# atenpas/gpd

Measured on AMD Instinct MI355X. Metric: 15-ch grasp candidates scored/sec (imagegen+LeNet) at 1/2/4/8 MI355X, higher is better.
Workload: dtype f64 geometry / u8 images / LeNet f32-equivalent by exact operand splitting: conv1 int8 digit planes of 32-bit fixed-point weights (i32 accumulate, exact), conv2 + ip1 three bf16 pieces per operand (six exact products per term, f32 accumulate), ip2 f32

## Files before the change

### gpd_amd/csrc/lenet_fast.hip

```cpp
#include "gpd_internal.h"
#include "buffers.h"

#include <cstring>

namespace gpd {

typedef int i32x4 __attribute__((ext_vector_type(4)));
typedef float f32x4 __attribute__((ext_vector_type(4)));
typedef __bf16 bf16x8 __attribute__((ext_vector_type(8)));
typedef unsigned int u32x4 __attribute__((ext_vector_type(4)));

constexpr int F1_THREADS = 512, F1_WAVES = 8;
constexpr int F1_PITCH = 72;
constexpr int F1_ROWB = F1_PITCH * 16;
constexpr int F1_HWC = kImg * F1_ROWB;
constexpr int F1_TILES = 28 * 7;
constexpr int F1_KS = 7, F1_MT = 5;

__host__ __device__ constexpr int f1_tap(int ks, int g) {
  return ks < 5 ? ((g == 0 ? 0 : g == 1 ? 2 : g == 2 ? 1 : 3) * 5 + ks) : ks == 5 ? 20 + g : (g == 0 ? 24 : -1);
}
constexpr int F1P_KS = 5;
constexpr int F1P_ROWB = 736;
constexpr int F1P_COPY = kImg * F1P_ROWB;
constexpr int F1N_KS = 3;
constexpr int F1N_PITCH = 68;
constexpr int F1N_COPY = kImg * F1N_PITCH * 4;
__host__ __device__ constexpr int f1n_slot(int ks, int g) {
  const int sl = 4 * ks + g;
  return sl < 5 ? 2 * sl : sl < 10 ? 2 * (sl - 5) + 1 : -1;
}

__device__ inline double max_f64(double a, double b) {
  double r;
  asm("v_max_f64 %0, %1, %2" : "=v"(r) : "v"(a), "v"(b));
  return r;
}
__device__ inline double dpp_quad_max(double v) {
  int lo = __double2loint(v), hi = __double2hiint(v);
  double o = __hiloint2double(__builtin_amdgcn_mov_dpp(hi, 0xB1, 0xf, 0xf, true), __builtin_amdgcn_mov_dpp(lo, 0xB1, 0xf, 0xf, true));
  v = max_f64(v, o);
  lo = __double2loint(v);
  hi = __double2hiint(v);
  o = __hiloint2double(__builtin_amdgcn_mov_dpp(hi, 0x4E, 0xf, 0xf, true), __builtin_amdgcn_mov_dpp(lo, 0x4E, 0xf, 0xf, true));
  return max_f64(v, o);
}

template <int C, bool RELU>
__device__ __forceinline__ void conv1_i8_body(const uint8_t *__restrict__ images, const uint4 *__restrict__ atab,
                                              const double *__restrict__ corr, const int *__restrict__ shift,
                                              const float *__restrict__ bias, float *__restrict__ pool1, int n,
                                              int *__restrict__ queue) {
  constexpr int RAW = C * kPix, NV = RAW / 16;
  static_assert(RAW % 16 == 0 && C <= 16, "image bytes");
  constexpr bool NARROW = C <= 4;
  constexpr bool PACK12 = C == 12;
  constexpr int KS = NARROW ? F1N_KS : PACK12 ? F1P_KS : F1_KS;
  __shared__ __attribute__((aligned(16))) uint8_t s_hwc[NARROW ? 4 * F1N_COPY : PACK12 ? 2 * F1P_COPY : F1_HWC];
  __shared__ __attribute__((aligned(16))) uint8_t s_raw[RAW];
  __shared__ int s_nxt;
  const int tid = threadIdx.x, lane = tid & 63;
  const int wave = __builtin_amdgcn_readfirstlane(tid >> 6);
  const int j = lane & 15, q = lane >> 4;
  int img = blockIdx.x;
  if (img >= n) return;
  if (wave < F1_WAVES / 2) __builtin_amdgcn_s_setprio(2);
  i32x4 A[KS][F1_MT];
#pragma unroll
  for (int ks = 0; ks < KS; ks++)
#pragma unroll
    for (int mt = 0; mt < F1_MT; mt++) {
      const uint4 v = atab[(ks * F1_MT + mt) * 64 + lane];
      A[ks][mt] = i32x4{(int)v.x, (int)v.y, (int)v.z, (int)v.w};
    }
  {
    const uint4 *src = reinterpret_cast<const uint4 *>(images + (size_t)img * RAW);
    uint4 *dst = reinterpret_cast<uint4 *>(s_raw);
    for (int i = tid; i < NV; i += F1_THREADS) dst[i] = src[i];
  }
  __syncthreads();
  auto transpose = [&]() {
    if constexpr (NARROW) {
      for (int task = tid; task < kImg * (kImg / 4); task += F1_THREADS) {
        const int y = task / (kImg / 4), x0 = 4 * (task - y * (kImg / 4));
        uint32_t r[4];
#pragma unroll
        for (int c = 0; c < 4; c++) r[c] = c < C ? *reinterpret_cast<const uint32_t *>(s_raw + c * kPix + y * kImg + x0) : 0x80808080u;
        const uint32_t t0 = __builtin_amdgcn_perm(r[1], r[0], 0x05010400u), t1 = __builtin_amdgcn_perm(r[1], r[0], 0x07030602u);
        const uint32_t t2 = __builtin_amdgcn_perm(r[3], r[2], 0x05010400u), t3 = __builtin_amdgcn_perm(r[3], r[2], 0x07030602u);
        const uint32_t o0 = __builtin_amdgcn_perm(t2, t0, 0x05040100u) ^ 0x80808080u, o1 = __builtin_amdgcn_perm(t2, t0, 0x07060302u) ^ 0x80808080u;
        const uint32_t o2 = __builtin_amdgcn_perm(t3, t1, 0x05040100u) ^ 0x80808080u, o3 = __builtin_amdgcn_perm(t3, t1, 0x07060302u) ^ 0x80808080u;
        uint8_t *d = s_hwc + (y * F1N_PITCH + x0) * 4;
        *reinterpret_cast<uint4 *>(d) = make_uint4(o0, o1, o2, o3);
#pragma unroll
        for (int sh = 1; sh < 4; sh++) {
          uint32_t *e = reinterpret_cast<uint32_t *>(d + sh * F1N_COPY + sh * 4);
          e[0] = o0;
          e[1] = o1;
          e[2] = o2;
          e[3] = o3;
        }
      }
      return;
    }
    if constexpr (PACK12) {
      for (int task = tid; task < kImg * (kImg / 4); task += F1_THREADS) {
        const int y = task / (kImg / 4), x0 = 4 * (task - y * (kImg / 4));
        uint32_t o[4][3];
#pragma unroll
        for (int cg = 0; cg < 3; cg++) {
          uint32_t r[4];
#pragma unroll
          for (int c = 0; c < 4; c++) r[c] = *reinterpret_cast<const uint32_t *>(s_raw + (4 * cg + c) * kPix + y * kImg + x0);
          const uint32_t t0 = __builtin_amdgcn_perm(r[1], r[0], 0x05010400u), t1 = __builtin_amdgcn_perm(r[1], r[0], 0x07030602u);
          const uint32_t t2 = __builtin_amdgcn_perm(r[3], r[2], 0x05010400u), t3 = __builtin_amdgcn_perm(r[3], r[2], 0x07030602u);
          o[0][cg] = __builtin_amdgcn_perm(t2, t0, 0x05040100u) ^ 0x80808080u;
          o[1][cg] = __builtin_amdgcn_perm(t2, t0, 0x07060302u) ^ 0x80808080u;
          o[2][cg] = __builtin_amdgcn_perm(t3, t1, 0x05040100u) ^ 0x80808080u;
          o[3][cg] = __builtin_amdgcn_perm(t3, t1, 0x07060302u) ^ 0x80808080u;
        }
        uint8_t *d = s_hwc + y * F1P_ROWB + 12 * x0;
        uint4 *d4 = reinterpret_cast<uint4 *>(d);
        d4[0] = make_uint4(o[0][0], o[0][1], o[0][2], o[1][0]);
        d4[1] = make_uint4(o[1][1], o[1][2], o[2][0], o[2][1]);
        d4[2] = make_uint4(o[2][2], o[3][0], o[3][1], o[3][2]);
        uint32_t *e = reinterpret_cast<uint32_t *>(d + F1P_COPY + 4);
#pragma unroll
        for (int px = 0; px < 4; px++)
#pragma unroll
          for (int cg = 0; cg < 3; cg++) e[3 * px + cg] = o[px][cg];
      }
      return;
    }
    for (int task = tid; task < kImg * (kImg / 4); task += F1_THREADS) {
      const int y = task / (kImg / 4), x0 = 4 * (task - y * (kImg / 4));
      uint32_t r[16];
#pragma unroll
      for (int c = 0; c < 16; c++) r[c] = c < C ? *reinterpret_cast<const uint32_t *>(s_raw + c * kPix + y * kImg + x0) : 0u;
      uint32_t o[4][4];
#pragma unroll
      for (int cg = 0; cg < 4; cg++) {
        const uint32_t t0 = __builtin_amdgcn_perm(r[4 * cg + 1], r[4 * cg], 0x05010400u);
        const uint32_t t1 = __builtin_amdgcn_perm(r[4 * cg + 1], r[4 * cg], 0x07030602u);
        const uint32_t t2 = __builtin_amdgcn_perm(r[4 * cg + 3], r[4 * cg + 2], 0x05010400u);
        const uint32_t t3 = __builtin_amdgcn_perm(r[4 * cg + 3], r[4 * cg + 2], 0x07030602u);
        o[0][cg] = __builtin_amdgcn_perm(t2, t0, 0x05040100u) ^ 0x80808080u;
        o[1][cg] = __builtin_amdgcn_perm(t2, t0, 0x07060302u) ^ 0x80808080u;
        o[2][cg] = __builtin_amdgcn_perm(t3, t1, 0x05040100u) ^ 0x80808080u;
        o[3][cg] = __builtin_amdgcn_perm(t3, t1, 0x07060302u) ^ 0x80808080u;
      }
#pragma unroll
      for (int e = 0; e < 4; e++)
        *reinterpret_cast<uint4 *>(s_hwc + (y * F1_PITCH + x0 + e) * 16) = make_uint4(o[e][0], o[e][1], o[e][2], o[e][3]);
    }
  };
  transpose();
  const int m_row = (j >> 1) & 1, m_x = 2 * (j >> 2) + (j & 1);
  const int kyg = q == 0 ? 0 : q == 1 ? 2 : q == 2 ? 1 : 3;
  const int n_shift = (4 - (m_x & 3)) & 3;
  const int lane_off = NARROW   ? n_shift * F1N_COPY + (m_row * F1N_PITCH + m_x + n_shift) * 4
                       : PACK12 ? (m_x & 1) * (F1P_COPY + 4) + m_row * F1P_ROWB + 12 * m_x + 16 * q
                                : (m_row * F1_PITCH + m_x) * 16;
  int n_slot[F1N_KS];
#pragma unroll
  for (int ks = 0; ks < F1N_KS; ks++) {
    const int sl = q == 0 ? f1n_slot(ks, 0) : q == 1 ? f1n_slot(ks, 1) : q == 2 ? f1n_slot(ks, 2) : f1n_slot(ks, 3);
    n_slot[ks] = sl < 0 ? 0 : ((sl >> 1) * F1N_PITCH + 4 * (sl & 1)) * 4;
  }
  const int p = j & 3, w = j >> 2;
  const double k_corr_own = corr[4 * p + q], k_corr_4 = corr[16 + q];
  const int k_shift_own = shift[4 * p + q], k_shift_4 = shift[16 + q];
  const float k_bias_own = bias[4 * p + q], k_bias_4 = bias[16 + q];
  for (;;) {
    if (tid == 0) s_nxt = (int)gridDim.x + atomicAdd(queue, 1);
    __syncthreads();
    const int nxt = s_nxt;
    const uint4 *nsrc = reinterpret_cast<const uint4 *>(images + (size_t)(nxt < n ? nxt : img) * RAW);
    auto tile_addr = [&](int t, const uint8_t *&pa, const uint8_t *&pb, const uint8_t *&pc) {
      const int tc = t < F1_TILES ? t : F1_TILES - 1;
      const int trow = tc / 7, tcol = tc - 7 * trow;
      if constexpr (NARROW) {
        pa = pb = pc = s_hwc + ((2 * trow) * F1N_PITCH + 8 * tcol) * 4 + lane_off;
      } else if constexpr (PACK12) {
        pa = pb = pc = s_hwc + (2 * trow) * F1P_ROWB + 12 * (8 * tcol) + lane_off;
      } else {
        const uint8_t *base = s_hwc + ((2 * trow) * F1_PITCH + 8 * tcol) * 16 + lane_off;
        pa = base + kyg * F1_ROWB;
        pb = base + 4 * F1_ROWB + q * 16;
        pc = base + 4 * F1_ROWB + 4 * 16;
      }
    };
    auto frag_b = [&](int ks, const uint8_t *pa, const uint8_t *pb, const uint8_t *pc) {
      if constexpr (NARROW) return *reinterpret_cast<const i32x4 *>(pa + n_slot[ks < F1N_KS ? ks : 0]);
      else if constexpr (PACK12) {
        typedef const volatile __attribute__((address_space(3))) unsigned long long *lds_u64;
        const unsigned long long lo = *(lds_u64)(pa + ks * F1P_ROWB), hi = *(lds_u64)(pa + ks * F1P_ROWB + 8);
        return i32x4{(int)(uint32_t)lo, (int)(uint32_t)(lo >> 32), (int)(uint32_t)hi, (int)(uint32_t)(hi >> 32)};
      }
      else return *reinterpret_cast<const i32x4 *>(ks < 5 ? pa + ks * 16 : ks == 5 ? pb : pc);
    };
    i32x4 B[KS];
    {
      const uint8_t *pa, *pb, *pc;
      tile_addr(wave, pa, pb, pc);
#pragma unroll
      for (int ks = 0; ks < KS; ks++) B[ks] = frag_b(ks, pa, pb, pc);
    }
    int it = 0;
    for (int t = wave; t < F1_TILES; t += F1_WAVES, it++) {
      const int piece = it * F1_THREADS + tid;
      const bool has_piece = nxt < n && piece < NV;
      uint4 stage = make_uint4(0, 0, 0, 0);
      if (has_piece) stage = nsrc[piece];
      i32x4 acc[F1_MT];
#pragma unroll
      for (int mt = 0; mt < F1_MT; mt++) acc[mt] = i32x4{0, 0, 0, 0};
      __builtin_amdgcn_sched_barrier(0);
#pragma unroll
      for (int ks = 0; ks < KS; ks++)
#pragma unroll
        for (int mt = 0; mt < F1_MT; mt++) acc[mt] = __builtin_amdgcn_mfma_i32_16x16x64_i8(A[ks][mt], B[ks], acc[mt], 0, 0, 0);
      __builtin_amdgcn_sched_barrier(0);
      {
        const uint8_t *pa, *pb, *pc;
        tile_addr(t + F1_WAVES, pa, pb, pc);
#pragma unroll
        for (int ks = 0; ks < KS; ks++) B[ks] = frag_b(ks, pa, pb, pc);
      }
      __builtin_amdgcn_sched_barrier(0);
      double sm[F1_MT];
#pragma unroll
      for (int mt = 0; mt < F1_MT; mt++) {
        const int hi = (int)((unsigned)acc[mt][3] << 8) + acc[mt][2];
        const int lo = (int)((unsigned)acc[mt][1] << 8) + acc[mt][0];
        sm[mt] = dpp_quad_max(__builtin_fma((double)hi, 65536.0, (double)lo));
      }
      const double s_own = p == 0 ? sm[0] : p == 1 ? sm[1] : p == 2 ? sm[2] : sm[3];
      float v_own = ldexpf((float)(s_own + k_corr_own), -k_shift_own) + k_bias_own;
      float v_4 = ldexpf((float)(sm[4] + k_corr_4), -k_shift_4) + k_bias_4;
      if constexpr (RELU) {
        v_own = fmaxf(v_own, 0.f);
        v_4 = fmaxf(v_4, 0.f);
      }
      const int trow = t / 7, tcol = t - 7 * trow;
      float *dst = pool1 + ((size_t)img * 784 + trow * 28 + 4 * tcol + w) * 20;
      dst[4 * p + q] = v_own;
      if (p == 0) dst[16 + q] = v_4;
      if (has_piece) reinterpret_cast<uint4 *>(s_raw)[piece] = stage;
    }
    __syncthreads();
    if (nxt >= n) break;
    transpose();
    img = nxt;
  }
}

template <int C>
__global__ __launch_bounds__(F1_THREADS) void conv1_i8_kernel(const uint8_t *__restrict__ images,
                                                              const uint4 *__restrict__ atab, const double *__restrict__ corr,
                                                              const int *__restrict__ shift, const float *__restrict__ bias,
                                                              float *__restrict__ pool1, int n, int *__restrict__ queue) {
  conv1_i8_body<C, false>(images, atab, corr, shift, bias, pool1, n, queue);
}
template <int C>
__global__ __launch_bounds__(F1_THREADS) void conv1_i8_relu_kernel(const uint8_t *__restrict__ images,
                                                                   const uint4 *__restrict__ atab,
                                                                   const double *__restrict__ corr,
                                                                   const int *__restrict__ shift,
                                                                   const float *__restrict__ bias, float *__restrict__ pool1,
                                                                   int n, int *__restrict__ queue) {
  conv1_i8_body<C, true>(images, atab, corr, shift, bias, pool1, n, queue);
}

__device__ inline bf16x8 as_bf16x8(const uint4 &v) {
  bf16x8 r;
  __builtin_memcpy(&r, &v, 16);
  return r;
}

struct Bf3 {
  unsigned short h, m, l;
};
__host__ __device__ inline unsigned short bf16_bits(float x) {
#if defined(__HIP_DEVICE_COMPILE__)
  const __bf16 b = (__bf16)x;
  unsigned short u;
  __builtin_memcpy(&u, &b, 2);
  return u;
#else
  uint32_t u;
  memcpy(&u, &x, 4);
  if ((u & 0x7f800000u) == 0x7f800000u) return (unsigned short)((u >> 16) | ((u & 0xffffu) ? 0x40u : 0u));
  u += 0x7fffu + ((u >> 16) & 1u);
  return (unsigned short)(u >> 16);
#endif
}
__host__ __device__ inline float bf16_value(unsigned short b) {
  const uint32_t u = (uint32_t)b << 16;
  float f;
#if defined(__HIP_DEVICE_COMPILE__)
  __builtin_memcpy(&f, &u, 4);
#else
  memcpy(&f, &u, 4);
#endif
  return f;
}
__host__ __device__ inline Bf3 bf16_split3(float a) {
  Bf3 r;
  r.h = bf16_bits(a);
  const float r1 = a - bf16_value(r.h);
  r.m = bf16_bits(r1);
  const float r2 = r1 - bf16_value(r.m);
  r.l = bf16_bits(r2);
  return r;
}

constexpr int F2_THREADS = 512;
constexpr int F2_PP = 28 * 40;
constexpr int F2_RS = 3 * F2_PP;
constexpr int F2_IMG = 28 * F2_RS;
constexpr int F2_RAW = 784 * 20 * 4;
constexpr int F2_LUNITS = 24;
constexpr int F2_XLD = kLenetXld;

constexpr int F3_KSTEPS = F2_XLD / 32;
__host__ __device__ inline size_t f3_blocked(int r, int k, int pc) {
  const int rr = r & 15;
  return ((((size_t)(r >> 4) * F3_KSTEPS + (k >> 5)) * 3 + pc) << 10) + rr * 64 + ((((k >> 3) & 3) ^ ((4 - (rr >> 2)) & 3)) << 4) + (k & 7) * 2;
}

__host__ __device__ constexpr int f2_slot_tap(int e, int g) {
  return e < 25 ? (e / 5) * 5 + g : e < 30 ? g * 5 + 4 : e == 30 ? 24 : (g == 0 ? 24 : -1);
}
__host__ __device__ constexpr int f2_slot_cg(int e, int g) { return e < 25 ? e % 5 : e < 30 ? e - 25 : e == 30 ? g : 4; }

template <bool RELU>
__device__ __forceinline__ void conv2_bf16_body(const float *__restrict__ pool1, const uint4 *__restrict__ btab,
                                                const float *__restrict__ bias, unsigned short *__restrict__ xs, int n,
                                                int *__restrict__ queue) {
  __shared__ __attribute__((aligned(16))) uint8_t s_img[F2_IMG];
  __shared__ __attribute__((aligned(16))) uint8_t s_raw[F2_RAW];
  __shared__ int s_nxt;
  const int tid = threadIdx.x, lane = tid & 63;
  const int wave = __builtin_amdgcn_readfirstlane(tid >> 6);
  const int j = lane & 15, q = lane >> 4;
  const int img0 = blockIdx.x;
  if (img0 >= n) return;
  {
    const uint4 *src = reinterpret_cast<const uint4 *>(pool1 + (size_t)img0 * (784 * 20));
    uint4 *dst = reinterpret_cast<uint4 *>(s_raw);
    for (int i = tid; i < F2_RAW / 16; i += F2_THREADS) dst[i] = src[i];
  }
  __syncthreads();
  auto split = [&]() {
    for (int task = tid; task < 784 * 5; task += F2_THREADS) {
      const int px = task / 5, cg = task - 5 * px;
      const int row = px / 28, col = px - 28 * row;
      const float4 a = *reinterpret_cast<const float4 *>(s_raw + px * 80 + cg * 16);
      const Bf3 s0 = bf16_split3(a.x), s1 = bf16_split3(a.y), s2 = bf16_split3(a.z), s3 = bf16_split3(a.w);
      uint8_t *d = s_img + row * F2_RS + col * 40 + cg * 8;
      *reinterpret_cast<uint2 *>(d) = make_uint2(s0.h | ((uint32_t)s1.h << 16), s2.h | ((uint32_t)s3.h << 16));
      *reinterpret_cast<uint2 *>(d + F2_PP) = make_uint2(s0.m | ((uint32_t)s1.m << 16), s2.m | ((uint32_t)s3.m << 16));
      *reinterpret_cast<uint2 *>(d + 2 * F2_PP) = make_uint2(s0.l | ((uint32_t)s1.l << 16), s2.l | ((uint32_t)s3.l << 16));
    }
  };
  split();
  auto store_x = [&](int img, int pixel, int f, float v) {
    const Bf3 sp = bf16_split3(v);
    uint8_t *o = reinterpret_cast<uint8_t *>(xs) + f3_blocked(img, pixel * 50 + f, 0);
    *reinterpret_cast<unsigned short *>(o) = sp.h;
    *reinterpret_cast<unsigned short *>(o + 1024) = sp.m;
    *reinterpret_cast<unsigned short *>(o + 2048) = sp.l;
  };
  auto image_loop = [&](int passes, auto carries, auto &&work) {
    int img = img0;
    for (;;) {
      if (tid == 0) s_nxt = (int)gridDim.x + atomicAdd(queue, 1);
      __syncthreads();
      const int nxt = s_nxt;
      const uint4 *nsrc = reinterpret_cast<const uint4 *>(pool1 + (size_t)(nxt < n ? nxt : img) * (784 * 20));
#pragma unroll 1
      for (int tt = 0; tt < passes; tt++) {
        const int piece = tt * (7 * 64) + tid;
        const bool has_piece = decltype(carries)::value && nxt < n && piece < F2_RAW / 16;
        uint4 stage = make_uint4(0, 0, 0, 0);
        if (has_piece) stage = nsrc[piece];
        work(img, tt);
        if (has_piece) reinterpret_cast<uint4 *>(s_raw)[piece] = stage;
      }
      __syncthreads();
      if (nxt >= n) break;
      split();
      img = nxt;
    }
  };
  if (wave == 7) {
    __builtin_amdgcn_s_setprio(3);
    bf16x8 LW[3][4];
#pragma unroll
    for (int pc = 0; pc < 3; pc++)
#pragma unroll
      for (int ks = 0; ks < 4; ks++) LW[pc][ks] = as_bf16x8(btab[((3 * 3 + pc) * 16 + ks) * 64 + lane]);
    int l_lo[4], l_hi[4];
#pragma unroll
    for (int ks = 0; ks < 4; ks++) {
      const int idx = min(4 * ks + q, 14), ky = idx / 3, c8 = idx - 3 * ky;
      l_lo[ks] = ky * F2_RS + j * 40 + c8 * 16;
      l_hi[ks] = c8 == 2 ? l_lo[ks] : l_lo[ks] + 8;
    }
    const int f_own = 48 + (q & 1);
    const float k_bias = bias[f_own];
    auto unit_base = [&](int u) { return s_img + (2 * (u >> 1)) * F2_RS + (12 * (u & 1)) * 40; };
    auto lfrag = [&](const uint8_t *ubase, int step, int pc) -> bf16x8 {
      typedef const volatile __attribute__((address_space(3))) unsigned long long *lds_u64;
      const uint8_t *a = ubase + (step >> 2) * F2_RS + pc * F2_PP;
      const unsigned long long lo = *(lds_u64)(a + l_lo[step & 3]), hi = *(lds_u64)(a + l_hi[step & 3]);
      return as_bf16x8(make_uint4((uint32_t)lo, (uint32_t)(lo >> 32), (uint32_t)hi, (uint32_t)(hi >> 32)));
    };
    bf16x8 b_buf[4][3];
    auto shl = [](float v, auto n) {
      return __builtin_bit_cast(float, __builtin_amdgcn_update_dpp(0, __builtin_bit_cast(int, v), 0x100 + decltype(n)::value, 0xf, 0xf, true));
    };
    asm volatile("" ::"v"(k_bias));
    image_loop(F2_LUNITS, std::false_type(), [&](int img, int tt) {
      const uint8_t *ubase = unit_base(tt), *unext = unit_base(tt < F2_LUNITS - 1 ? tt + 1 : tt);
      if (tt == 0) {
#pragma unroll
        for (int st = 0; st < 3; st++)
#pragma unroll
          for (int pc = 0; pc < 3; pc++) b_buf[st][pc] = lfrag(ubase, st, pc);
      }
      f32x4 lacc[2][2] = {{f32x4{0.f, 0.f, 0.f, 0.f}, f32x4{0.f, 0.f, 0.f, 0.f}}, {f32x4{0.f, 0.f, 0.f, 0.f}, f32x4{0.f, 0.f, 0.f, 0.f}}};
#pragma unroll
      for (int step = 0; step < 8; step++) {
#pragma unroll
        for (int pc = 0; pc < 3; pc++) b_buf[(step + 3) & 3][pc] = step + 3 < 8 ? lfrag(ubase, step + 3, pc) : lfrag(unext, step + 3 - 8, pc);
#pragma unroll
        for (int term = 0; term < 6; term++) {
          const int pa = term == 0 ? 2 : (term == 2 || term == 3) ? 1 : 0;
          const int pw = term == 1 ? 2 : (term == 2 || term == 4) ? 1 : 0;
          lacc[step >> 2][term & 1] = __builtin_amdgcn_mfma_f32_16x16x32_bf16(LW[pw][step & 3], b_buf[step & 3][pa], lacc[step >> 2][term & 1], 0, 0, 0);
        }
      }
      float conv_row[2];
#pragma unroll
      for (int rr = 0; rr < 2; rr++) {
        const f32x4 t = lacc[rr][0] + lacc[rr][1];
        const float v = ((t[0] + shl(t[1], std::integral_constant<int, 1>())) + shl(t[2], std::integral_constant<int, 2>())) + shl(t[3], std::integral_constant<int, 3>());
        conv_row[rr] = v + __shfl(shl(t[0], std::integral_constant<int, 4>()), (lane + 32) & 63);
      }
      float pv = fmaxf(conv_row[0], conv_row[1]);
      pv = fmaxf(pv, shl(pv, std::integral_constant<int, 1>())) + k_bias;
      if constexpr (RELU) pv = fmaxf(pv, 0.f);
      if (q < 2 && (j & 1) == 0 && j < 12) store_x(img, (tt >> 1) * 12 + 6 * (tt & 1) + (j >> 1), f_own, pv);
    });
    return;
  }
  const int grp = wave < 4 ? 1 + (wave >> 1) : 0;
  const int t0 = wave == 3 ? 20 : wave < 4 ? 18 * (wave & 1) : 12 * (wave - 4), tcnt = wave == 2 ? 20 : wave == 3 ? 16 : wave < 4 ? 18 : 12;
  bf16x8 W[3][16];
#pragma unroll
  for (int pc = 0; pc < 3; pc++)
#pragma unroll
    for (int ks = 0; ks < 16; ks++) W[pc][ks] = as_bf16x8(btab[((grp * 3 + pc) * 16 + ks) * 64 + lane]);
  const int m_row = (j >> 1) & 1, m_x = 2 * (j >> 2) + (j & 1);
  const int lane_off = m_row * F2_RS + m_x * 40;
  const int off_x = lane_off + 40 * q, off_y = lane_off + q * F2_RS + 4 * 40, off_z = lane_off + 4 * F2_RS + 4 * 40 + 8 * q,
            off_w = lane_off + 4 * F2_RS + 4 * 40 + 32;
  const int f_own = 16 * grp + j;
  const float k_bias = bias[f_own];
  auto tile_base = [&](int tt) {
    const int T = t0 + tt, rp = T / 3, xt = T - 3 * rp;
    return s_img + (2 * rp) * F2_RS + (8 * xt) * 40;
  };
  auto frag = [&](const uint8_t *base, int ks, int pc) -> bf16x8 {
    uint2 v[2];
#pragma unroll
    for (int h = 0; h < 2; h++) {
      const int e = ks + 16 * h;
      const uint8_t *a = e < 25 ? base + off_x + (e / 5) * F2_RS + (e % 5) * 8
                         : e < 30 ? base + off_y + (e - 25) * 8
                         : e == 30 ? base + off_z
                                   : base + off_w;
      typedef const volatile __attribute__((address_space(3))) unsigned long long *lds_u64;
      const unsigned long long t = *(lds_u64)(a + pc * F2_PP);
      v[h] = make_uint2((uint32_t)t, (uint32_t)(t >> 32));
    }
    return as_bf16x8(make_uint4(v[0].x, v[0].y, v[1].x, v[1].y));
  };
  bf16x8 a_buf[2][3];
  image_loop(tcnt, std::true_type(), [&](int img, int tt) {
    if (tt == 0) {
#pragma unroll
      for (int pc = 0; pc < 3; pc++) a_buf[0][pc] = frag(tile_base(0), 0, pc);
    }
    const int T = t0 + tt, rp = T / 3, xt = T - 3 * rp;
    const uint8_t *base = tile_base(tt), *base_next = tile_base(tt < tcnt - 1 ? tt + 1 : tt);
    f32x4 acc[2] = {f32x4{0.f, 0.f, 0.f, 0.f}, f32x4{0.f, 0.f, 0.f, 0.f}};
#pragma unroll
    for (int ks = 0; ks < 16; ks++) {
#pragma unroll
      for (int pc = 0; pc < 3; pc++) a_buf[(ks + 1) & 1][pc] = ks + 1 < 16 ? frag(base, ks + 1, pc) : frag(base_next, 0, pc);
#pragma unroll
      for (int term = 0; term < 6; term++) {
        const int pa = term == 0 ? 2 : (term == 2 || term == 3) ? 1 : 0;
        const int pw = term == 1 ? 2 : (term == 2 || term == 4) ? 1 : 0;
        acc[term & 1] = __builtin_amdgcn_mfma_f32_16x16x32_bf16(a_buf[ks & 1][pa], W[pw][ks], acc[term & 1], 0, 0, 0);
      }
    }
    const f32x4 t = acc[0] + acc[1];
    float pv = fmaxf(fmaxf(t[0], t[1]), fmaxf(t[2], t[3])) + k_bias;
    if constexpr (RELU) pv = fmaxf(pv, 0.f);
    store_x(img, rp * 12 + 4 * xt + q, f_own, pv);
  });
}

__global__ __launch_bounds__(F2_THREADS) void conv2_bf16_kernel(const float *__restrict__ pool1,
                                                                const uint4 *__restrict__ btab, const float *__restrict__ bias,
                                                                unsigned short *__restrict__ xs, int n,
                                                                int *__restrict__ queue) {
  conv2_bf16_body<false>(pool1, btab, bias, xs, n, queue);
}
__global__ __launch_bounds__(F2_THREADS) void conv2_bf16_relu_kernel(const float *__restrict__ pool1,
                                                                     const uint4 *__restrict__ btab,
                                                                     const float *__restrict__ bias,
                                                                     unsigned short *__restrict__ xs, int n,
                                                                     int *__restrict__ queue) {
  conv2_bf16_body<true>(pool1, btab, bias, xs, n, queue);
}

constexpr int F3_THREADS = 512, F3_BN = 256, F3_BK = 32, F3_KQ = 4;
constexpr int F3_KLEN = F2_XLD / F3_KQ, F3_STEPS = F3_KLEN / F3_BK;
static_assert(F2_XLD % (F3_KQ * F3_BK) == 0 && F2_XLD >= kFc1In, "K quarters");
static_assert(F3_STEPS % 2 == 1, "the step loop below runs in pairs + one");

typedef const __attribute__((address_space(1))) void *glds_src_t;
typedef __attribute__((address_space(3))) void *glds_dst_t;

template <int NT>
__global__ __launch_bounds__(F3_THREADS) void fc1_bf16_kernel(const unsigned short *__restrict__ xs, const unsigned short *__restrict__ wt,
                                                             float *__restrict__ out_p, int n) {
  constexpr int BM = 32 * NT;
  constexpr int XB = BM * 64, WB = F3_BN * 64;
  constexpr int STAGE = 3 * (XB + WB);
  __shared__ __attribute__((aligned(16))) uint8_t smem_a[STAGE];
  __shared__ __attribute__((aligned(16))) uint8_t smem_b[STAGE];
  static_assert(2 * STAGE <= 160 * 1024, "LDS");
  const int tid = threadIdx.x;
  const int L = blockIdx.x;
  const int xcd = L & 7;
  const int ut = xcd & 1, kq = xcd >> 1;
  const int m0 = (L >> 3) * BM;
  if (m0 >= n) return;
  const int u0 = ut * F3_BN, k_base = kq * F3_KLEN;
  const int wave = __builtin_amdgcn_readfirstlane(tid >> 6), lane = tid & 63;
  const int wm = wave >> 2, wu = wave & 3;
  const int g = lane >> 4, j = lane & 15;
  constexpr int XBLK = 6 * NT, X_PW = (XBLK + 7) / 8;
  constexpr size_t ROWBLK = (size_t)F3_KSTEPS * 3 * 1024;
  const uint8_t *wsrc[2];
#pragma unroll
  for (int i = 0; i < 2; i++)
    wsrc[i] = reinterpret_cast<const uint8_t *>(wt) + (size_t)(u0 / 16 + wave + 8 * i) * ROWBLK + (size_t)(k_base / 32) * 3072 + lane * 16;
  const uint8_t *xsrc[X_PW];
  int xdst[X_PW];
#pragma unroll
  for (int i = 0; i < X_PW; i++) {
    const int e = min(wave + 8 * i, XBLK - 1), rb = e / 3, pc = e - 3 * rb;
    xsrc[i] = reinterpret_cast<const uint8_t *>(xs) + (size_t)min(m0 / 16 + rb, (n - 1) / 16) * ROWBLK + (size_t)(k_base / 32) * 3072 + pc * 1024 + lane * 16;
    xdst[i] = pc * XB + rb * 1024;
  }
  auto fetch = [&](int step, uint8_t *b) {
    const int so = step * 3072;
#pragma unroll
    for (int pc = 0; pc < 3; pc++)
#pragma unroll
      for (int i = 0; i < 2; i++)
        __builtin_amdgcn_global_load_lds((glds_src_t)(wsrc[i] + so + pc * 1024), (glds_dst_t)(b + 3 * XB + pc * WB + (wave + 8 * i) * 1024), 16, 0, 0);
#pragma unroll
    for (int i = 0; i < X_PW; i++)
      if (wave + 8 * i < XBLK) __builtin_amdgcn_global_load_lds((glds_src_t)(xsrc[i] + so), (glds_dst_t)(b + xdst[i]), 16, 0, 0);
  };
  f32x4 acc[NT][4];
#pragma unroll
  for (int t = 0; t < NT; t++)
#pragma unroll
    for (int c = 0; c < 4; c++) acc[t][c] = f32x4{0.f, 0.f, 0.f, 0.f};
  const int foff = j * 64 + ((g ^ ((4 - (j >> 2)) & 3)) << 4);
  const int xoff = (wm * 16 * NT) * 64 + foff, woff = (wu * 64) * 64 + foff;
  auto compute = [&](const uint8_t *b) {
    bf16x8 wb[3][4], xa[2][NT];
    auto ldw = [&](int pc) {
#pragma unroll
      for (int c = 0; c < 4; c++) wb[pc][c] = as_bf16x8(*reinterpret_cast<const uint4 *>(b + 3 * XB + pc * WB + woff + c * 16 * 64));
    };
    auto ldx = [&](int s, int pa) {
#pragma unroll
      for (int t = 0; t < NT; t++) xa[s][t] = as_bf16x8(*reinterpret_cast<const uint4 *>(b + pa * XB + xoff + t * 16 * 64));
    };
    auto mul = [&](int s, int pw) {
#pragma unroll
      for (int t = 0; t < NT; t++)
#pragma unroll
        for (int c = 0; c < 4; c++) acc[t][c] = __builtin_amdgcn_mfma_f32_16x16x32_bf16(xa[s][t], wb[pw][c], acc[t][c], 0, 0, 0);
    };
    ldw(0);
    ldx(0, 2);
    ldw(1);
    ldx(1, 1);
    __builtin_amdgcn_sched_barrier(0);
    mul(0, 0);
    __builtin_amdgcn_sched_barrier(0);
    ldw(2);
    ldx(0, 0);
    __builtin_amdgcn_sched_barrier(0);
    mul(1, 1);
    mul(1, 0);
    __builtin_amdgcn_sched_barrier(0);
    mul(0, 2);
    mul(0, 1);
    mul(0, 0);
  };
  fetch(0, smem_a);
  __syncthreads();
  for (int t = 0; t < F3_STEPS - 1; t += 2) {
    fetch(t + 1, smem_b);
    __builtin_amdgcn_sched_barrier(0);
    compute(smem_a);
    __syncthreads();
    fetch(t + 2, smem_a);
    __builtin_amdgcn_sched_barrier(0);
    compute(smem_b);
    __syncthreads();
  }
  compute(smem_a);
#pragma unroll
  for (int c = 0; c < 4; c++) {
    const int u = u0 + 64 * wu + 16 * c + j;
    if (u >= kFc1Out) continue;
#pragma unroll
    for (int t = 0; t < NT; t++) {
      const int m = m0 + 16 * NT * wm + 16 * t + 4 * g;
      if (m < n) *reinterpret_cast<f32x4 *>(out_p + fc1p_index(m, kq, u)) = acc[t][c];
    }
  }
}

void lenet_fast_free(LeNetFast &f) {
  device_release(f.c1a, f.c1corr, f.c1shift, f.c2b, f.f1wt);
  f = LeNetFast();
}

void lenet_fast_conv1_tables(int channels, const float *w, std::vector<uint8_t> &atab, std::vector<double> &corr, std::vector<int> &shift) {
  const int K = channels * 25;
  std::vector<long long> W((size_t)20 * K);
  corr.assign(20, 0.0);
  shift.assign(20, 0);
  for (int f = 0; f < 20; f++) {
    float mx = 0.f;
    for (int k = 0; k < K; k++) mx = std::fmax(mx, std::fabs(w[(size_t)f * K + k]));
    int s = 0;
    if (mx > 0.f) {
      int e;
      (void)std::frexp(mx, &e);
      s = 30 - e;
    }
    shift[f] = s;
    long long sum = 0;
    for (int k = 0; k < K; k++) {
      const long long v = std::llrint(std::ldexp((double)w[(size_t)f * K + k], s));
      W[(size_t)f * K + k] = v;
      sum += v;
    }
    corr[f] = 128.0 * (double)sum;
  }
  atab.assign((size_t)F1_KS * F1_MT * 64 * 16, 0);
  auto digit_of = [](long long v, int digit) {
    int d = 0;
    for (int q = 0; q <= digit; q++) {
      d = (int)(((v + 128) & 255) - 128);
      v = (v - d) >> 8;
    }
    return d;
  };
  const bool narrow = channels <= 4;
  const bool pack12 = channels == 12;
  for (int ks = 0; ks < (narrow ? F1N_KS : pack12 ? F1P_KS : F1_KS); ks++)
    for (int mt = 0; mt < F1_MT; mt++)
      for (int lane = 0; lane < 64; lane++) {
        const int i = lane & 15, g = lane >> 4;
        const int f = 4 * mt + (i >> 2), digit = i & 3;
        uint8_t *row = &atab[((size_t)(ks * F1_MT + mt) * 64 + lane) * 16];
        if (narrow) {
          const int sl = f1n_slot(ks, g);
          if (sl < 0) continue;
          const int ky = sl >> 1, half = sl & 1;
          for (int px = 0; px < 4; px++) {
            const int kx = 4 * half + px;
            if (kx > 4) continue;
            for (int c = 0; c < channels; c++) row[4 * px + c] = (uint8_t)(int8_t)digit_of(W[(size_t)f * K + c * 25 + ky * 5 + kx], digit);
          }
          continue;
        }
        if (pack12) {
          for (int b = 0; b < 16; b++) {
            const int kb = 16 * g + b;
            if (kb >= 60) continue;
            row[b] = (uint8_t)(int8_t)digit_of(W[(size_t)f * K + (kb % 12) * 25 + ks * 5 + kb / 12], digit);
          }
          continue;
        }
        const int tap = f1_tap(ks, g);
        if (tap < 0) continue;
        for (int c = 0; c < channels; c++) row[c] = (uint8_t)(int8_t)digit_of(W[(size_t)f * K + c * 25 + tap], digit);
      }
}

void lenet_fast_conv2_tables(const float *w, std::vector<unsigned short> &btab) {
  btab.assign((size_t)4 * 3 * 16 * 64 * 8, 0);
  auto put = [&](int slot, int ks, int lane, int e, float v) {
    const Bf3 sp = bf16_split3(v);
    const unsigned short pcs[3] = {sp.h, sp.m, sp.l};
    for (int pc = 0; pc < 3; pc++) btab[((((size_t)slot * 3 + pc) * 16 + ks) * 64 + lane) * 8 + e] = pcs[pc];
  };
  for (int slot = 0; slot < 3; slot++)
    for (int ks = 0; ks < 16; ks++)
      for (int lane = 0; lane < 64; lane++) {
        const int f = 16 * slot + (lane & 15), g = lane >> 4;
        for (int h = 0; h < 2; h++) {
          const int e = ks + 16 * h, tap = f2_slot_tap(e, g), cg = f2_slot_cg(e, g);
          if (tap < 0) continue;
          for (int c = 0; c < 4; c++) put(slot, ks, lane, 4 * h + c, w[(size_t)f * 500 + (4 * cg + c) * 25 + tap]);
        }
      }
  for (int ks = 0; ks < 4; ks++)
    for (int lane = 0; lane < 64; lane++) {
      const int row = lane & 15, chunk = 4 * ks + (lane >> 4);
      if ((row > 8 && row != 12) || chunk > 14) continue;
      const int f = row < 8 ? 48 + (row >> 2) : 48 + ((row - 8) >> 2), kx = row < 8 ? (row & 3) : 4;
      const int ky = chunk / 3, c0 = 8 * (chunk % 3);
      for (int e = 0; e < 8 && c0 + e < 20; e++) put(3, ks, lane, e, w[(size_t)f * 500 + (c0 + e) * 25 + ky * 5 + kx]);
    }
}

void lenet_fast_ip1_tables(const float *w, std::vector<unsigned short> &wt) {
  wt.assign((size_t)3 * 512 * F2_XLD, 0);
  uint8_t *base = reinterpret_cast<uint8_t *>(wt.data());
  for (int k = 0; k < kFc1In; k++)
    for (int u = 0; u < kFc1Out; u++) {
      const Bf3 sp = bf16_split3(w[(size_t)k * kFc1Out + u]);
      const unsigned short pcs[3] = {sp.h, sp.m, sp.l};
      for (int pc = 0; pc < 3; pc++) memcpy(base + f3_blocked(u, k, pc), &pcs[pc], 2);
    }
}

void lenet_fast_unblock_x(const unsigned short *blocked, int n, unsigned short *planes) {
  const uint8_t *base = reinterpret_cast<const uint8_t *>(blocked);
  for (int pc = 0; pc < 3; pc++)
    for (int m = 0; m < n; m++)
      for (int k = 0; k < kFc1In; k++) memcpy(planes + ((size_t)pc * n + m) * kFc1In + k, base + f3_blocked(m, k, pc), 2);
}

}

extern "C" int gpd_hip_lenet_fast_tables(int channels, const float *c1w, const float *c2w, uint8_t *atab, double *corr, int *shift,
                                         unsigned short *btab) {
  if (!c1w || !c2w || !atab || !corr || !shift || !btab || channels < 1 || channels > 16) return GPD_ERR_INVALID;
  std::vector<uint8_t> a;
  std::vector<double> c;
  std::vector<int> sh;
  std::vector<unsigned short> b;
  gpd::lenet_fast_conv1_tables(channels, c1w, a, c, sh);
  gpd::lenet_fast_conv2_tables(c2w, b);
  memcpy(atab, a.data(), a.size());
  memcpy(corr, c.data(), c.size() * sizeof(double));
  memcpy(shift, sh.data(), sh.size() * sizeof(int));
  memcpy(btab, b.data(), b.size() * sizeof(unsigned short));
  return GPD_OK;
}

namespace gpd {

hipError_t lenet_fast_prepare(LeNetFast &f, int channels, const float *c1w, const float *c2w, const float *f1w) {
  lenet_fast_free(f);
  std::vector<uint8_t> atab;
  std::vector<double> corr;
  std::vector<int> shift;
  std::vector<unsigned short> btab, wt;
  lenet_fast_conv1_tables(channels, c1w, atab, corr, shift);
  lenet_fast_conv2_tables(c2w, btab);
  lenet_fast_ip1_tables(f1w, wt);
  hipError_t e;
  auto up = [&](auto *&dst, const void *src, size_t bytes) -> hipError_t {
    if ((e = device_alloc(dst, (bytes + sizeof(*dst) - 1) / sizeof(*dst))) != hipSuccess) return e;
    return hipMemcpy(dst, src, bytes, hipMemcpyHostToDevice);
  };
  if ((e = up(f.c1a, atab.data(), atab.size())) != hipSuccess) return e;
  if ((e = up(f.c1corr, corr.data(), corr.size() * sizeof(double))) != hipSuccess) return e;
  if ((e = up(f.c1shift, shift.data(), shift.size() * sizeof(int))) != hipSuccess) return e;
  if ((e = up(f.c2b, btab.data(), btab.size() * sizeof(unsigned short))) != hipSuccess) return e;
  if ((e = up(f.f1wt, wt.data(), wt.size() * sizeof(unsigned short))) != hipSuccess) return e;
  return hipSuccess;
}

template <int NT>
static void fc1f_launch(const LeNetWeights &w, LeNetScratch &s, int n, hipStream_t stream) {
  const int m_tiles = (n + 32 * NT - 1) / (32 * NT);
  fc1_bf16_kernel<NT><<<m_tiles * 8, F3_THREADS, 0, stream>>>(s.xs, w.fast.f1wt, s.fc1p, n);
}
static int fc1f_pick_nt(int n) {
  for (int r = 1;; r++) {
    const int nt = (n + 32 * r * 32 - 1) / (32 * r * 32);
    if (nt <= 5) return nt < 1 ? 1 : nt;
  }
}

hipError_t lenet_forward_fast(const LeNetWeights &w, LeNetScratch &s, const uint8_t *img, int m, float *d_scores, hipStream_t stream,
                              hipEvent_t *kernel_events, int *queue) {
  const int num_cus = s.num_cus;
  const int grid = m < num_cus ? m : num_cus;
#define F1_LAUNCH(KERNEL, CH) KERNEL<CH><<<grid, F1_THREADS, 0, stream>>>(img, w.fast.c1a, w.fast.c1corr, w.fast.c1shift, w.c1b, s.pool1, m, queue)
  if (w.conv_relu) {
    switch (w.channels) {
      case 15: F1_LAUNCH(conv1_i8_relu_kernel, 15); break;
      case 12: F1_LAUNCH(conv1_i8_relu_kernel, 12); break;
      case 3: F1_LAUNCH(conv1_i8_relu_kernel, 3); break;
      case 1: F1_LAUNCH(conv1_i8_relu_kernel, 1); break;
      default: return hipErrorInvalidValue;
    }
  } else {
    switch (w.channels) {
      case 15: F1_LAUNCH(conv1_i8_kernel, 15); break;
      case 12: F1_LAUNCH(conv1_i8_kernel, 12); break;
      case 3: F1_LAUNCH(conv1_i8_kernel, 3); break;
      case 1: F1_LAUNCH(conv1_i8_kernel, 1); break;
      default: return hipErrorInvalidValue;
    }
  }
#undef F1_LAUNCH
  if (kernel_events) (void)hipEventRecord(kernel_events[0], stream);
  if (w.conv_relu)
    conv2_bf16_relu_kernel<<<grid, F2_THREADS, 0, stream>>>(s.pool1, w.fast.c2b, w.c2b, s.xs, m, queue + 1);
  else
    conv2_bf16_kernel<<<grid, F2_THREADS, 0, stream>>>(s.pool1, w.fast.c2b, w.c2b, s.xs, m, queue + 1);
  if (kernel_events) (void)hipEventRecord(kernel_events[1], stream);
  switch (fc1f_pick_nt(m)) {
    case 1: fc1f_launch<1>(w, s, m, stream); break;
    case 2: fc1f_launch<2>(w, s, m, stream); break;
    case 3: fc1f_launch<3>(w, s, m, stream); break;
    case 4: fc1f_launch<4>(w, s, m, stream); break;
    default: fc1f_launch<5>(w, s, m, stream); break;
  }
  if (kernel_events) (void)hipEventRecord(kernel_events[2], stream);
  return hipGetLastError();
}

}
```

Before: 2.284 million.

## Stream conv2 next-image input via direct global-to-LDS loads and interleave MFMA with LDS reads

The next image's pool1 data is now prefetched with global_load_lds_dwordx4 straight into LDS, one 64-lane chunk per wave per pass, instead of staging it through registers and storing it afterwards. A single vmcnt wait sits before the barrier. The conv2 and tail-wave inner loops now use explicit sched_group_barrier interleaving of MFMAs with LDS reads, plus reordered fragment loads so that single-buffered mid/low pieces are reused as soon as they are consumed. Tile counts between waves 2 and 3 are rebalanced and the first-fragment preload is hoisted into a per-image callback. This relies on inline asm that sets m0 and on scheduling hints, so register pressure and correctness depend on the exact chunk bounds.

```diff
diff --git a/gpd_amd/csrc/lenet_fast.hip b/gpd_amd/csrc/lenet_fast.hip
--- a/gpd_amd/csrc/lenet_fast.hip
+++ b/gpd_amd/csrc/lenet_fast.hip
@@ -372,22 +372,29 @@
     *reinterpret_cast<unsigned short *>(o + 1024) = sp.m;
     *reinterpret_cast<unsigned short *>(o + 2048) = sp.l;
   };
-  auto image_loop = [&](int passes, auto carries, auto &&work) {
+  auto image_loop = [&](int passes, auto carries, auto &&first, auto &&work) {
     int img = img0;
     for (;;) {
       if (tid == 0) s_nxt = (int)gridDim.x + atomicAdd(queue, 1);
       __syncthreads();
+      first();
       const int nxt = s_nxt;
       const uint4 *nsrc = reinterpret_cast<const uint4 *>(pool1 + (size_t)(nxt < n ? nxt : img) * (784 * 20));
 #pragma unroll 1
       for (int tt = 0; tt < passes; tt++) {
-        const int piece = tt * (7 * 64) + tid;
-        const bool has_piece = decltype(carries)::value && nxt < n && piece < F2_RAW / 16;
-        uint4 stage = make_uint4(0, 0, 0, 0);
-        if (has_piece) stage = nsrc[piece];
+        const int chunk = tt * 7 + wave;
+        if (decltype(carries)::value && __builtin_amdgcn_readfirstlane(nxt) < n && chunk < (F2_RAW / 16 + 63) / 64) {
+          typedef __attribute__((address_space(3))) void *lds_ptr_t;
+          const int p0 = min(chunk * 64, F2_RAW / 16 - 64);
+          const unsigned dst = __builtin_amdgcn_readfirstlane((unsigned)(unsigned long)(lds_ptr_t)(s_raw + p0 * 16));
+#pragma clang diagnostic push
+#pragma clang diagnostic ignored "-Winline-asm"
+          asm volatile("s_mov_b32 m0, %0\n\ts_nop 0\n\tglobal_load_lds_dwordx4 %1, off" ::"s"(dst), "v"(nsrc + p0 + lane) : "memory", "m0");
+#pragma clang diagnostic pop
+        }
         work(img, tt);
-        if (has_piece) reinterpret_cast<uint4 *>(s_raw)[piece] = stage;
-      }
+      }
+      if (decltype(carries)::value) asm volatile("s_waitcnt vmcnt(0)" ::: "memory");
       __syncthreads();
       if (nxt >= n) break;
       split();
@@ -422,14 +429,14 @@
       return __builtin_bit_cast(float, __builtin_amdgcn_update_dpp(0, __builtin_bit_cast(int, v), 0x100 + decltype(n)::value, 0xf, 0xf, true));
     };
     asm volatile("" ::"v"(k_bias));
-    image_loop(F2_LUNITS, std::false_type(), [&](int img, int tt) {
+    auto lfirst = [&]() {
+#pragma unroll
+      for (int st = 0; st < 3; st++)
+#pragma unroll
+        for (int pc = 0; pc < 3; pc++) b_buf[st][pc] = lfrag(unit_base(0), st, pc);
+    };
+    image_loop(F2_LUNITS, std::false_type(), lfirst, [&](int img, int tt) {
       const uint8_t *ubase = unit_base(tt), *unext = unit_base(tt < F2_LUNITS - 1 ? tt + 1 : tt);
-      if (tt == 0) {
-#pragma unroll
-        for (int st = 0; st < 3; st++)
-#pragma unroll
-          for (int pc = 0; pc < 3; pc++) b_buf[st][pc] = lfrag(ubase, st, pc);
-      }
       f32x4 lacc[2][2] = {{f32x4{0.f, 0.f, 0.f, 0.f}, f32x4{0.f, 0.f, 0.f, 0.f}}, {f32x4{0.f, 0.f, 0.f, 0.f}, f32x4{0.f, 0.f, 0.f, 0.f}}};
 #pragma unroll
       for (int step = 0; step < 8; step++) {
@@ -441,13 +448,24 @@
           const int pw = term == 1 ? 2 : (term == 2 || term == 4) ? 1 : 0;
           lacc[step >> 2][term & 1] = __builtin_amdgcn_mfma_f32_16x16x32_bf16(LW[pw][step & 3], b_buf[step & 3][pa], lacc[step >> 2][term & 1], 0, 0, 0);
         }
-      }
+        __builtin_amdgcn_sched_group_barrier(0x100, 2, 0);
+        __builtin_amdgcn_sched_group_barrier(0x008, 1, 0);
+        __builtin_amdgcn_sched_group_barrier(0x100, 2, 0);
+        __builtin_amdgcn_sched_group_barrier(0x008, 1, 0);
+        __builtin_amdgcn_sched_group_barrier(0x100, 2, 0);
+        __builtin_amdgcn_sched_group_barrier(0x008, 4, 0);
+      }
+      __builtin_amdgcn_sched_barrier(0);
       float conv_row[2];
-#pragma unroll
-      for (int rr = 0; rr < 2; rr++) {
-        const f32x4 t = lacc[rr][0] + lacc[rr][1];
-        const float v = ((t[0] + shl(t[1], std::integral_constant<int, 1>())) + shl(t[2], std::integral_constant<int, 2>())) + shl(t[3], std::integral_constant<int, 3>());
-        conv_row[rr] = v + __shfl(shl(t[0], std::integral_constant<int, 4>()), (lane + 32) & 63);
+      {
+        const f32x4 ta = lacc[0][0] + lacc[0][1], tb = lacc[1][0] + lacc[1][1];
+        const float xa = __shfl(shl(ta[0], std::integral_constant<int, 4>()), (lane + 32) & 63);
+        const float xb = __shfl(shl(tb[0], std::integral_constant<int, 4>()), (lane + 32) & 63);
+        __builtin_amdgcn_sched_barrier(0);
+        const float va = ((ta[0] + shl(ta[1], std::integral_constant<int, 1>())) + shl(ta[2], std::integral_constant<int, 2>())) + shl(ta[3], std::integral_constant<int, 3>());
+        const float vb = ((tb[0] + shl(tb[1], std::integral_constant<int, 1>())) + shl(tb[2], std::integral_constant<int, 2>())) + shl(tb[3], std::integral_constant<int, 3>());
+        conv_row[0] = va + xa;
+        conv_row[1] = vb + xb;
       }
       float pv = fmaxf(conv_row[0], conv_row[1]);
       pv = fmaxf(pv, shl(pv, std::integral_constant<int, 1>())) + k_bias;
@@ -457,7 +475,7 @@
     return;
   }
   const int grp = wave < 4 ? 1 + (wave >> 1) : 0;
-  const int t0 = wave == 3 ? 20 : wave < 4 ? 18 * (wave & 1) : 12 * (wave - 4), tcnt = wave == 2 ? 20 : wave == 3 ? 16 : wave < 4 ? 18 : 12;
+  const int t0 = wave == 3 ? 19 : wave < 4 ? 18 * (wave & 1) : 12 * (wave - 4), tcnt = wave == 2 ? 19 : wave == 3 ? 17 : wave < 4 ? 18 : 12;
   bf16x8 W[3][16];
 #pragma unroll
   for (int pc = 0; pc < 3; pc++)
@@ -488,25 +506,35 @@
     }
     return as_bf16x8(make_uint4(v[0].x, v[0].y, v[1].x, v[1].y));
   };
-  bf16x8 a_buf[2][3];
-  image_loop(tcnt, std::true_type(), [&](int img, int tt) {
-    if (tt == 0) {
-#pragma unroll
-      for (int pc = 0; pc < 3; pc++) a_buf[0][pc] = frag(tile_base(0), 0, pc);
-    }
+  bf16x8 a_h[2], a_m, a_l;
+  auto first = [&]() {
+    a_l = frag(tile_base(0), 0, 2);
+    a_m = frag(tile_base(0), 0, 1);
+    a_h[0] = frag(tile_base(0), 0, 0);
+  };
+  image_loop(tcnt, std::true_type(), first, [&](int img, int tt) {
     const int T = t0 + tt, rp = T / 3, xt = T - 3 * rp;
     const uint8_t *base = tile_base(tt), *base_next = tile_base(tt < tcnt - 1 ? tt + 1 : tt);
     f32x4 acc[2] = {f32x4{0.f, 0.f, 0.f, 0.f}, f32x4{0.f, 0.f, 0.f, 0.f}};
 #pragma unroll
     for (int ks = 0; ks < 16; ks++) {
-#pragma unroll
-      for (int pc = 0; pc < 3; pc++) a_buf[(ks + 1) & 1][pc] = ks + 1 < 16 ? frag(base, ks + 1, pc) : frag(base_next, 0, pc);
-#pragma unroll
-      for (int term = 0; term < 6; term++) {
-        const int pa = term == 0 ? 2 : (term == 2 || term == 3) ? 1 : 0;
-        const int pw = term == 1 ? 2 : (term == 2 || term == 4) ? 1 : 0;
-        acc[term & 1] = __builtin_amdgcn_mfma_f32_16x16x32_bf16(a_buf[ks & 1][pa], W[pw][ks], acc[term & 1], 0, 0, 0);
-      }
+      const uint8_t *nb = ks + 1 < 16 ? base : base_next;
+      const int nk = (ks + 1) & 15;
+      a_h[(ks + 1) & 1] = frag(nb, nk, 0);
+      acc[0] = __builtin_amdgcn_mfma_f32_16x16x32_bf16(a_l, W[0][ks], acc[0], 0, 0, 0);
+      a_l = frag(nb, nk, 2);
+      acc[1] = __builtin_amdgcn_mfma_f32_16x16x32_bf16(a_h[ks & 1], W[2][ks], acc[1], 0, 0, 0);
+      acc[0] = __builtin_amdgcn_mfma_f32_16x16x32_bf16(a_m, W[1][ks], acc[0], 0, 0, 0);
+      acc[1] = __builtin_amdgcn_mfma_f32_16x16x32_bf16(a_m, W[0][ks], acc[1], 0, 0, 0);
+      a_m = frag(nb, nk, 1);
+      acc[0] = __builtin_amdgcn_mfma_f32_16x16x32_bf16(a_h[ks & 1], W[1][ks], acc[0], 0, 0, 0);
+      acc[1] = __builtin_amdgcn_mfma_f32_16x16x32_bf16(a_h[ks & 1], W[0][ks], acc[1], 0, 0, 0);
+      __builtin_amdgcn_sched_group_barrier(0x100, 2, 0);
+      __builtin_amdgcn_sched_group_barrier(0x008, 1, 0);
+      __builtin_amdgcn_sched_group_barrier(0x100, 2, 0);
+      __builtin_amdgcn_sched_group_barrier(0x008, 3, 0);
+      __builtin_amdgcn_sched_group_barrier(0x100, 2, 0);
+      __builtin_amdgcn_sched_group_barrier(0x008, 2, 0);
     }
     const f32x4 t = acc[0] + acc[1];
     float pv = fmaxf(fmaxf(t[0], t[1]), fmaxf(t[2], t[3])) + k_bias;
```

New measurement: 2.306 million (median of 6 runs). Within noise of the previous version (+1.0%).
